# aosokin/os2d

Measured on AMD Instinct MI355X. Metric: query-image-pairs/s (1280-px input, ResNet50, N-class), higher is better.
Workload: dtype fftx3 (as fft; the per-bin complex GEMM on the fp16 MFMA with spectra split into fp16 hi+lo, 3 MFMAs per product, fp32 accumulate)

## Files before the change

os2d_amd/csrc/dft_mfma.h:

```cpp
#pragma once

#ifndef DFT_DEV
#error "the includer defines DFT_DEV, DFT_TID, DFT_BID, DFT_GRID, DFT_LDS, DFT_BARRIER, DFT_MFMA, DFT_SHFL_XOR, DFT_SHFL_XOR_U32, DFT_BALLOT, DFT_FLAG, DFT_FLAG_SET, DFT_RAISE, DFT_UNIFORM"
#endif

#ifndef DFT_HD
#define DFT_HD static inline
#endif
#ifndef DFT_MEMBER
#define DFT_MEMBER inline
#endif
#ifndef DFT_LANDED
#define DFT_LANDED(X)
#endif
#ifndef DFT_FWD_PREFETCH_AFTER
#define DFT_FWD_PREFETCH_AFTER 2
#endif
#ifndef DFT_INV_PREFETCH_AFTER
#define DFT_INV_PREFETCH_AFTER 2
#endif
#ifndef DFT_PIPE_REGA
#define DFT_PIPE_REGA 1
#endif
#ifndef DFT_PIPE_LDS
#define DFT_PIPE_LDS 1
#endif
#ifndef DFT_SCHED_FENCE
#define DFT_SCHED_FENCE()
#endif
#ifndef DFT_STREAM_STORE
#define DFT_STREAM_STORE(P, V) (*(P) = (V))
#endif
#ifndef DFT_STAMP
#define DFT_STAMP(K)
#define DFT_STAMP_BEGIN()
#define DFT_STAMP_END(BASE)
#endif

#include "tile_common.h"

namespace os2d_dft {

typedef float f32x4u __attribute__((ext_vector_type(4), aligned(4)));

constexpr int DFT_THR = 512, DFT_WAVES = 8;
constexpr int DFT_G = 4;
constexpr int DFT_MAXP = 64;
constexpr int DFT_MAXV = 48;
constexpr int DFT_MAXWK = 96;
constexpr int DFT_KREG = 8;
constexpr int DFT_OUT_SHB = 0, DFT_OUT_SHB_BORDERS = 1, DFT_OUT_PLANES = 2;

struct DftPlan {
  int H, W;
  int P, Q, V, NBINS;
  int T, TY, TX, TH, TW;
  int oy, ox;
  int LH, LW;
  int RH;
  int Pp;
  int Wk;
  int N1;
  int M2;
  int Mx;
  int N2;
  int MA;
  int MB;
  int KB;
  int NBo;
  int G;
  int eT;
  int fast;
  unsigned inv_cg, inv_t, inv_tx, inv_c4, inv_v, inv_pq, inv_og, inv_kg, inv_pp;
  int lds_const, lds_union, lds_total;
};

DFT_HD int dft_round_up(int x, int m) { return (x + m - 1) / m * m; }
DFT_HD unsigned dft_magic(unsigned d) { return d > 1 ? (unsigned)(((1ull << 32) + d - 1) / d) : 0u; }

DFT_HD int dft_units_fqt(int P, int Q) { return (dft_round_up(Q, 16) / 8) * 2 * dft_round_up(Q + 2, 32); }
constexpr int DFT_R2_P = 64, DFT_R2_MATU = 8 * 2 * 64, DFT_R2_TWU = 16;
constexpr int DFT_R2_LDS_TW = 512;
DFT_HD bool dft_radix2(int P) { return P == DFT_R2_P; }
DFT_HD int dft_units_fp2(int P, int Q) {
  return dft_radix2(P) ? DFT_R2_MATU + DFT_R2_TWU : (2 * dft_round_up(P, 8) / 8) * 2 * dft_round_up(2 * P, 32);
}
DFT_HD int dft_units_e2(int P, int Q) { return (2 * dft_round_up(P, 8) / 8) * 2 * dft_round_up(2 * P, 32); }
DFT_HD int dft_units_gq(int P, int Q) { return (dft_round_up(Q + 2, 16) / 8) * 2 * dft_round_up(Q, 32); }
DFT_HD size_t dft_matrices_units(int P, int Q) {
  return (size_t)dft_units_fqt(P, Q) + dft_units_fp2(P, Q) + dft_units_e2(P, Q) + dft_units_gq(P, Q);
}

static inline bool dft_plan_transform(int LH, int LW, int RH, int ncols, int minP, int minQ, int G, DftPlan* pl) {
  pl->G = G;
  pl->P = dft_round_up(minP, 4);
  if (pl->P == 60) pl->P = DFT_R2_P;
  pl->Q = dft_round_up(minQ, 2);
  pl->V = pl->Q / 2 + 1;
  pl->NBINS = dft_round_up(pl->P * pl->V, 8);
  pl->LH = LH;
  pl->LW = LW;
  pl->RH = RH;
  pl->Pp = dft_round_up(pl->P, 8);
  pl->Wk = dft_round_up(LW, 16);
  pl->N1 = dft_round_up(2 * pl->V, 32);
  pl->M2 = dft_round_up(2 * pl->P, 32);
  pl->Mx = dft_round_up(G * pl->Pp, 32);
  pl->N2 = dft_round_up(G * pl->V, 32);
  pl->MA = dft_round_up(2 * RH, 32);
  pl->MB = G * (pl->MA / 2);
  pl->KB = dft_round_up(2 * pl->V, 16);
  pl->NBo = dft_round_up(ncols, 32);
  int e = 0;
  while ((1 << e) < pl->P) ++e;
  pl->eT = e + 1;
  if (pl->P > DFT_MAXP || pl->V > DFT_MAXV || pl->Wk > DFT_MAXWK || LH > pl->P || LW > pl->Q || RH > pl->P) return false;
  const int fqt = (pl->Wk / 8) * 2 * pl->N1 * 16, gq = (pl->KB / 8) * 2 * pl->NBo * 16;
  const int x = (pl->Wk / 8) * 2 * (pl->Mx + 1) * 16, r2 = (2 * pl->Pp / 8) * 2 * (pl->N2 + 1) * 16;
  const int xs = pl->V * (pl->P * 8 * G + 16);
  const int y2 = r2, tt = (pl->KB / 8) * 2 * (pl->MB + 1) * 16;
  int u = x;
  if (r2 > u) u = r2;
  if (xs > u) u = xs;
  if (y2 > u) u = y2;
  if (tt > u) u = tt;
  if (G == 8) {
    if (dft_radix2(pl->P)) return false;
    const int fp2 = (2 * pl->Pp / 8) * 2 * pl->M2 * 16;
    const int ca = fqt + fp2, cb = gq + fp2;
    pl->lds_const = ca > cb ? ca : cb;
    pl->lds_union = dft_round_up(u, 256);
    pl->lds_total = pl->lds_const + pl->lds_union + 1024;
    const int t1 = (pl->Mx / 32) * (pl->N1 / 32), t2 = (pl->M2 / 32) * (pl->N2 / 32), tA = (pl->MA / 32) * (pl->N2 / 32),
              tB = (pl->MB / 32) * (pl->NBo / 32);
    const int npos = pl->Pp * (pl->Wk / 4), nitem = G * pl->V * (pl->Pp / 8);
    return pl->lds_total <= 160 * 1024 && t1 <= 24 && t2 <= 24 && tA <= 24 && tB <= 24 && npos <= 2 * DFT_THR && nitem <= 3 * DFT_THR;
  }
  pl->lds_const = fqt > gq ? fqt : gq;
  pl->lds_union = dft_round_up(u, 256);
  pl->lds_total = pl->lds_const + pl->lds_union + 1024;
  return pl->lds_total <= 160 * 1024;
}

static inline void dft_set_tiles(DftPlan* pl, int H, int W, int TY, int TX, int TH, int TW) {
  pl->H = H;
  pl->W = W;
  pl->TY = TY;
  pl->TX = TX;
  pl->T = TY * TX;
  pl->TH = TH;
  pl->TW = TW;
  pl->oy = TY > 1 ? 3 : 0;
  pl->ox = TX > 1 ? 3 : 0;
  pl->fast = (pl->T == 1 && (W & 3) == 0) ? 1 : 0;
  pl->inv_t = dft_magic((unsigned)pl->T);
  pl->inv_tx = dft_magic((unsigned)TX);
  pl->inv_c4 = dft_magic((unsigned)(pl->Wk / 4));
  pl->inv_v = dft_magic((unsigned)pl->V);
  pl->inv_pq = dft_magic((unsigned)(pl->P / 4 * pl->G * 2));
  pl->inv_kg = dft_magic((unsigned)(pl->Pp / 8));
  pl->inv_pp = dft_magic((unsigned)pl->Pp);
}

struct DftSize {
  int P, Q;
};
// ... 63 lines not shown
  *hi = __builtin_bit_cast(u32x2, h);
#ifdef DFT_SPLIT_LO_PAIR
  u32x2 l;
  l[0] = DFT_SPLIT_LO_PAIR(a, b, (*hi)[0]);
  l[1] = DFT_SPLIT_LO_PAIR(c, d, (*hi)[1]);
  *lo = l;
#else
  const half4 l = __builtin_convertvector(x - __builtin_convertvector(h, f32x4), half4);
  *lo = __builtin_bit_cast(u32x2, l);
#endif
}

DFT_DEV half8 dft_frag(const u32x4* p) { return __builtin_bit_cast(half8, *p); }

DFT_DEV f32x16 dft_mma3(half8 ah, half8 al, half8 bh, half8 bl, f32x16 acc) {
  acc = DFT_MFMA(ah, bl, acc);
  acc = DFT_MFMA(al, bh, acc);
  acc = DFT_MFMA(ah, bh, acc);
  return acc;
}

template <int NT, int KS>
DFT_DEV void dft_product_rega(f32x16* acc, const half8* ah, const half8* al, int ksn, const u32x4* B, int bstride, int nt0,
                              int ntstep, int l31, int hw) {
  constexpr int KR = KS ? KS : DFT_KREG;
  half8 bh[2][NT], bl[2][NT];
#define DFT_REGA_READ(KSTEP, SET)                                                                                          \
  _Pragma("unroll") for (int j = 0; j < NT; ++j) {                                                                         \
    bh[SET][j] = dft_frag(B + (size_t)((2 * (KSTEP) + hw) * 2 + 0) * bstride + (nt0 + ntstep * j) * 32 + l31);             \
    bl[SET][j] = dft_frag(B + (size_t)((2 * (KSTEP) + hw) * 2 + 1) * bstride + (nt0 + ntstep * j) * 32 + l31);             \
  }
  if (DFT_PIPE_REGA) DFT_REGA_READ(0, 0)
#pragma unroll
  for (int ks = 0; ks < KR; ++ks) {
    if (KS || ks < ksn) {
      if (DFT_PIPE_REGA) {
        if (ks + 1 < KR && (KS || ks + 1 < ksn)) DFT_REGA_READ(ks + 1, (ks + 1) & 1)
        DFT_SCHED_FENCE();
      } else {
        DFT_REGA_READ(ks, ks & 1)
      }
#pragma unroll
      for (int j = 0; j < NT; ++j) acc[j] = dft_mma3(ah[ks], al[ks], bh[ks & 1][j], bl[ks & 1][j], acc[j]);
      if (DFT_PIPE_REGA) DFT_SCHED_FENCE();
    }
  }
#undef DFT_REGA_READ
}

template <int KS>
DFT_DEV void dft_product_rega_any(f32x16* acc, int ntiles, const half8* ah, const half8* al, int ksn, const u32x4* B, int bstride,
                                  int nt0, int ntstep, int l31, int hw) {
  if (ntiles == 3) dft_product_rega<3, KS>(acc, ah, al, ksn, B, bstride, nt0, ntstep, l31, hw);
  else if (ntiles == 2) dft_product_rega<2, KS>(acc, ah, al, ksn, B, bstride, nt0, ntstep, l31, hw);
  else if (ntiles == 1) dft_product_rega<1, KS>(acc, ah, al, ksn, B, bstride, nt0, ntstep, l31, hw);
}

template <int NT, bool SHARE, int NW, int PIPE_MODE>
DFT_DEV void dft_product_lds(f32x16* acc, int ks0, int ks1, const u32x4* A, int astride, const u32x4* B, int bstride, int t0, int mtn,
                             int l31, int hw) {
  constexpr int NA = SHARE ? 1 : NT;
  int tm[NT], tn[NT];
#pragma unroll
  for (int j = 0; j < NT; ++j) {
    const int t = t0 + NW * j;
    tn[j] = t / mtn;
    tm[j] = t - tn[j] * mtn;
  }
  half8 ah[2][NA], al[2][NA], bh[2][NT], bl[2][NT];
#define DFT_LDS_READ(KSTEP, SET)                                                                                           \
  {                                                                                                                        \
    const int kc_ = (KSTEP) < ks1 ? (KSTEP) : ks1 - 1;                                                                     \
    _Pragma("unroll") for (int j = 0; j < NA; ++j) {                                                                       \
      ah[SET][j] = dft_frag(A + (size_t)((2 * kc_ + hw) * 2 + 0) * astride + tm[j] * 32 + l31);                            \
      al[SET][j] = dft_frag(A + (size_t)((2 * kc_ + hw) * 2 + 1) * astride + tm[j] * 32 + l31);                            \
    }                                                                                                                      \
    _Pragma("unroll") for (int j = 0; j < NT; ++j) {                                                                       \
      bh[SET][j] = dft_frag(B + (size_t)((2 * kc_ + hw) * 2 + 0) * bstride + tn[j] * 32 + l31);                            \
      bl[SET][j] = dft_frag(B + (size_t)((2 * kc_ + hw) * 2 + 1) * bstride + tn[j] * 32 + l31);                            \
    }                                                                                                                      \
  }
#define DFT_LDS_MMA(SET)                                                                                                   \
  DFT_SCHED_FENCE();                                                                                                       \
  _Pragma("unroll") for (int j = 0; j < NT; ++j)                                                                           \
    acc[j] = dft_mma3(ah[SET][SHARE ? 0 : j], al[SET][SHARE ? 0 : j], bh[SET][j], bl[SET][j], acc[j]);                    \
  DFT_SCHED_FENCE();
  if (ks0 >= ks1) return;
  constexpr bool PIPE = PIPE_MODE == 2 || (PIPE_MODE == 1 && SHARE);
  if (!PIPE) {
    for (int ks = ks0; ks < ks1; ++ks) {
      DFT_LDS_READ(ks, 0)
      _Pragma("unroll") for (int j = 0; j < NT; ++j)
        acc[j] = dft_mma3(ah[0][SHARE ? 0 : j], al[0][SHARE ? 0 : j], bh[0][j], bl[0][j], acc[j]);
    }
    return;
  }
  DFT_LDS_READ(ks0, 0)
  int ks = ks0;
  for (; ks + 1 < ks1; ks += 2) {
    DFT_LDS_READ(ks + 1, 1)
    DFT_LDS_MMA(0)
    DFT_LDS_READ(ks + 2, 0)
    DFT_LDS_MMA(1)
  }
  if (ks < ks1) {
    DFT_LDS_MMA(0)
  }
#undef DFT_LDS_READ
#undef DFT_LDS_MMA
}

template <int NW, int PIPE_MODE>
DFT_DEV void dft_product_lds_any(f32x16* acc, int ntiles, int ks0, int ks1, const u32x4* A, int astride, const u32x4* B, int bstride,
                                 int t0, int mtn, int l31, int hw) {
  const bool share = mtn == NW;
  if (ntiles == 3) {
    if (share) dft_product_lds<3, true, NW, PIPE_MODE>(acc, ks0, ks1, A, astride, B, bstride, t0, mtn, l31, hw);
    else dft_product_lds<3, false, NW, PIPE_MODE>(acc, ks0, ks1, A, astride, B, bstride, t0, mtn, l31, hw);
  } else if (ntiles == 2) {
    if (share) dft_product_lds<2, true, NW, PIPE_MODE>(acc, ks0, ks1, A, astride, B, bstride, t0, mtn, l31, hw);
    else dft_product_lds<2, false, NW, PIPE_MODE>(acc, ks0, ks1, A, astride, B, bstride, t0, mtn, l31, hw);
  } else if (ntiles == 1) {
    dft_product_lds<1, true, NW, PIPE_MODE>(acc, ks0, ks1, A, astride, B, bstride, t0, mtn, l31, hw);
  }
}

DFT_DEV void dft_matrix_unit(int which, int unit, int P, int Q, const double* twP, const double* twQ, u32x4* out) {
  const int V = Q / 2 + 1;
  const bool r2 = which == 1 && dft_radix2(P);
  if (r2 && unit >= DFT_R2_MATU) {
    const int u = 2 * (unit - DFT_R2_MATU);
    u32x4 o;
    for (int t = 0; t < 4; ++t) o[t] = __builtin_bit_cast(unsigned, (float)twP[2 * u + t]);
    *out = o;
    return;
  }
  const int tws = r2 ? 2 : 1;
  if (r2) P /= 2;
  const int Pp = dft_round_up(P, 8);
  int cols, kidx, hl, col;
  double vals[8];
  if (which == 0) cols = dft_round_up(2 * V, 32);
  else if (which == 1 || which == 2) cols = dft_round_up(2 * P, 32);
  else cols = dft_round_up(Q, 32);
  col = unit % cols;
  hl = (unit / cols) & 1;
  kidx = unit / (2 * cols);
  for (int t = 0; t < 8; ++t) {
    const int k = kidx * 8 + t;
    double x = 0.0;
    if (which == 0) {
      const int v = col >> 1, ri = col & 1;
      if (k < Q && v < V) x = twQ[2 * (int)(((long long)v * k) % Q) + ri] * 16384.0;
    } else if (which == 1) {
      const int ri = k / Pp, h = k - ri * Pp, u = col >> 1, ro = col & 1;
      if (h < P && u < P && ri < 2) {
        const int a = (int)(((long long)u * h) % P) * tws;
        const double c = twP[2 * a], s = -twP[2 * a + 1];
        x = (ro == 0 ? (ri == 0 ? c : s) : (ri == 0 ? -s : c)) * 16384.0;
      }
    } else if (which == 2) {
      const int ri = k / Pp, u = k - ri * Pp, h = col >> 1, ro = col & 1;
      if (u < P && h < P && ri < 2) {
        const int a = (int)(((long long)u * h) % P);
        const double c = twP[2 * a], s = -twP[2 * a + 1];
        x = (ro == 0 ? (ri == 0 ? c : -s) : (ri == 0 ? s : c)) * 16384.0;
      }
    } else {
      const int v = k >> 1, ri = k & 1;
      if (v < V && col < Q) {
        const double a = (v == 0 || 2 * v == Q) ? 1.0 : 2.0;
        x = a * twQ[2 * (int)(((long long)v * col) % Q) + ri] * 8192.0;
      }
    }
    vals[t] = x;
  }
  unsigned w[4];
  for (int t = 0; t < 4; ++t) {
    unsigned short b[2];
    for (int e = 0; e < 2; ++e) {
      const double x = vals[2 * t + e];
      const _Float16 h = (_Float16)x;
      const _Float16 r = hl == 0 ? h : (_Float16)(x - (double)h);
      b[e] = __builtin_bit_cast(unsigned short, r);
    }
    w[t] = (unsigned)b[0] | ((unsigned)b[1] << 16);
  }
  u32x4 o;
  o[0] = w[0];
  o[1] = w[1];
  o[2] = w[2];
  o[3] = w[3];
  *out = o;
}

template <bool TILED, bool FAST, int G, int NW, int KS2 = 0>
DFT_DEV void dft_forward_body(const float* corr,
                              const float* invn,
                              float* X,
                              const u32x4* FqT, const u32x4* Fp2, const DftPlan& pl, int C, int Cpad, int NBT, int iters) {
  constexpr int THR = NW * 64;
  constexpr bool ALDS = G == 8;
  constexpr bool R2 = !ALDS && KS2 == 8;
  unsigned char* smem = DFT_LDS;
  const int tid = DFT_TID, lane = tid & 63, l31 = lane & 31, hw = lane >> 5;
  const int wv = DFT_UNIFORM(tid >> 6);
  const int P = pl.P, V = pl.V, Pp = pl.Pp, Wk = pl.Wk, N1 = pl.N1, Mx = pl.Mx, N2 = pl.N2, LH = pl.LH, LW = pl.LW, W = pl.W, H = pl.H;
  const int MxS = Mx + 1, N2S = N2 + 1;
  const int CG = (C + G - 1) / G, HW = H * W;
  const bool unit_norm = invn == nullptr;
  u32x4* ldsF = reinterpret_cast<u32x4*>(smem);
  u32x4* ldsU = reinterpret_cast<u32x4*>(smem + pl.lds_const);
  unsigned char* ldsUb = smem + pl.lds_const;
  const int nF = (Wk / 8) * 2 * N1;
  for (int i = tid; i < nF; i += THR) ldsF[i] = FqT[i];
  const unsigned char* ldsTw = smem + pl.lds_const + pl.lds_union + DFT_R2_LDS_TW;
  if (R2 && tid < DFT_R2_TWU) reinterpret_cast<u32x4*>(smem + pl.lds_const + pl.lds_union + DFT_R2_LDS_TW)[tid] = Fp2[DFT_R2_MATU + tid];
  u32x4* ldsP = ldsF + nF;
  if (ALDS)
    for (int i = tid; i < (2 * Pp / 8) * 2 * pl.M2; i += THR) ldsP[i] = Fp2[i];

  const int mt1n = Mx / 32, nt1n = N1 / 32, nt2n = N2 / 32, mt2n = pl.M2 / 32;
  const int ks1n = Wk / 16, ks2n = 2 * Pp / 16;
  const int mt2 = wv & 3;
  constexpr int KR2 = R2 ? 4 : KS2 ? KS2 : DFT_KREG;
  half8 fp2h[KR2], fp2l[KR2];
  if (R2) {
#pragma unroll
    for (int ks = 0; ks < KR2; ++ks) {
      fp2h[ks] = dft_frag(Fp2 + ((size_t)((2 * ks + hw) * 2 + 0)) * 64 + (mt2 & 1) * 32 + l31);
      fp2l[ks] = dft_frag(Fp2 + ((size_t)((2 * ks + hw) * 2 + 1)) * 64 + (mt2 & 1) * 32 + l31);
    }
  } else if (!ALDS) {
#pragma unroll
    for (int ks = 0; ks < KR2; ++ks) {
      const int kc = ks < ks2n ? ks : 0, mc = mt2 < mt2n ? mt2 : 0;
      fp2h[ks] = dft_frag(Fp2 + ((size_t)((2 * kc + hw) * 2 + 0)) * pl.M2 + mc * 32 + l31);
      fp2l[ks] = dft_frag(Fp2 + ((size_t)((2 * kc + hw) * 2 + 1)) * pl.M2 + mc * 32 + l31);
    }
  }
  if (!ALDS) {
#pragma unroll
    for (int ks = 0; ks < KR2; ++ks) {
      DFT_LANDED(fp2h[ks]);
      DFT_LANDED(fp2l[ks]);
    }
  }

  constexpr int NSLOT = ALDS ? 2 : 3 * 512 / THR;
  const int npos = Pp * (Wk / 4);
  f32x4 pc[NSLOT][G], pn[NSLOT];
#define DFT_FWD_ITER(IT)                                                                                     \
  const int pr_ = dft_div((IT), pl.inv_cg), cg_ = (IT)-pr_ * CG;                                             \
  const int nb_ = TILED ? dft_div(pr_, pl.inv_t) : pr_, tile_ = TILED ? pr_ - nb_ * pl.T : 0;               \
  const int ty_ = TILED ? dft_div(tile_, pl.inv_tx) : 0, tx_ = TILED ? tile_ - ty_ * pl.TX : 0;             \
  const int Y0 = TILED ? ty_ * pl.TH - pl.oy : 0, X0 = TILED ? tx_ * pl.TW - pl.ox : 0;                     \
  const int c0_ = cg_ * G;
#define DFT_FWD_POS(TID, S)                                                                                  \
  const int i_ = (TID) + (S)*THR;                                                                        \
  const int r_ = dft_div(i_, pl.inv_c4), c4_ = i_ - r_ * (Wk / 4);                                          \
  const int y_ = Y0 + r_, x_ = X0 + 4 * c4_;
#define DFT_FWD_PREFETCH(IT, TID) DFT_FWD_PREFETCH_SLOTS(IT, TID, 0, NSLOT)
#define DFT_FWD_PREFETCH_SLOTS(IT, TID, S0, S1)                                                              \
  {                                                                                                          \
    DFT_FWD_ITER(IT)                                                                                         \
     \
    const float* nrm_ = invn ? invn + (size_t)nb_ * HW : corr + ((size_t)nb_ * C + (c0_ < C ? c0_ : C - 1)) * HW; \
    _Pragma("unroll") for (int s = (S0); s < (S1); ++s) {                                                    \
      DFT_FWD_POS(TID, s)                                                                                    \
      if (FAST) {                                                                                            \
        const bool ok = i_ < npos && r_ < LH && 4 * c4_ < LW;                                                \
        const int off = ok ? y_ * W + x_ : 0;                                                                \
        pn[s] = *reinterpret_cast<const f32x4*>(nrm_ + off);                                                \
        _Pragma("unroll") for (int g = 0; g < G; ++g) {                                                  \
          const int c = c0_ + g < C ? c0_ + g : C - 1;                                                       \
          pc[s][g] = *reinterpret_cast<const f32x4*>(corr + ((size_t)nb_ * C + c) * HW + off);              \
        }                                                                                                    \
      } else {                                                                                               \
                                                                           \
        const bool rok = i_ < npos && r_ < LH && y_ >= 0 && y_ < H;                                          \
        const int off0 = y_ * W + x_;                                                                        \
        const bool vec = rok && off0 >= 0 && off0 + 3 < HW;                                                  \
        const int offv = vec ? off0 : 0;                                                                     \
        pn[s] = *reinterpret_cast<const f32x4u*>(nrm_ + offv);                                               \
        _Pragma("unroll") for (int g = 0; g < G; ++g) {                                                      \
          const int c = c0_ + g < C ? c0_ + g : C - 1;                                                       \
          pc[s][g] = *reinterpret_cast<const f32x4u*>(corr + ((size_t)nb_ * C + c) * HW + offv);             \
        }                                                                                                    \
        if (rok && !vec) {                                                                                   \
          _Pragma("unroll") for (int e = 0; e < 4; ++e) {                                                    \
            const bool ok = 4 * c4_ + e < LW && x_ + e >= 0 && x_ + e < W;                                   \
            const int off = ok ? y_ * W + x_ + e : 0;                                                        \
            pn[s][e] = nrm_[off];                                                                            \
            _Pragma("unroll") for (int g = 0; g < G; ++g) {                                                  \
              const int c = c0_ + g < C ? c0_ + g : C - 1;                                                   \
              pc[s][g][e] = corr[((size_t)nb_ * C + c) * HW + off];                                          \
            }                                                                                                \
          }                                                                                                  \
        }                                                                                                    \
      }                                                                                                      \
    }                                                                                                        \
  }
  const int first = (DFT_GRID & 7) == 0 ? (DFT_BID & 7) * (DFT_GRID >> 3) + (DFT_BID >> 3) : DFT_BID;
  if (first < iters) DFT_FWD_PREFETCH(first, tid)
  DFT_BARRIER();

  DFT_STAMP_BEGIN()
  for (int it = first; it < iters; it += DFT_GRID) {
    int tl = tid;
#ifndef OS2D_HOST_EMU
    asm volatile("" : "+v"(tl));
#endif
    const int lane = tl & 63, l31 = lane & 31, hw = lane >> 5;
    DFT_FWD_ITER(it)
    {
#pragma unroll
      for (int s = 0; s < NSLOT; ++s) {
        DFT_FWD_POS(tl, s)
        if (i_ < npos) {
          float nsc[4];
#pragma unroll
          for (int e = 0; e < 4; ++e) {
            const bool ok = FAST ? (r_ < LH && 4 * c4_ < LW) : (r_ < LH && y_ >= 0 && y_ < H && 4 * c4_ + e < LW && x_ + e >= 0 && x_ + e < W);
            nsc[e] = ok ? (unit_norm ? 32768.0f : pn[s][e] * 32768.0f) : 0.f;
          }
#pragma unroll
          for (int g = 0; g < G; ++g) {
            u32x2 hi = {0u, 0u}, lo = {0u, 0u};
            if (c0_ + g < C)
              dft_split4(fmaxf(pc[s][g][0], 0.f) * nsc[0], fmaxf(pc[s][g][1], 0.f) * nsc[1], fmaxf(pc[s][g][2], 0.f) * nsc[2],
                         fmaxf(pc[s][g][3], 0.f) * nsc[3], &hi, &lo);
            const int m = g * Pp + (R2 ? (r_ & 1) * 32 + (r_ >> 1) : r_);
            unsigned char* dst = ldsUb + ((size_t)((c4_ >> 1) * 2) * MxS + m) * 16 + (c4_ & 1) * 8;
            *reinterpret_cast<u32x2*>(dst) = hi;
            *reinterpret_cast<u32x2*>(dst + (size_t)MxS * 16) = lo;
          }
        }
      }
      for (int i = tid; i < (Mx - G * Pp) * (Wk / 8) * 2; i += THR) {
        const int m = G * Pp + i % (Mx - G * Pp), kh = i / (Mx - G * Pp);
        ldsU[(size_t)kh * MxS + m] = u32x4{0u, 0u, 0u, 0u};
      }
    }
    DFT_BARRIER();
    DFT_STAMP(0)

    f32x16 acc[3];
    int tm[3], tn[3];
    int nt1w = 0;
#pragma unroll
    for (int j = 0; j < 3; ++j) {
      const int t = wv + NW * j;
      const bool mine = t < mt1n * nt1n;
      tn[j] = mine ? t / mt1n : 0;
      tm[j] = mine ? t - tn[j] * mt1n : -1;
      nt1w += mine ? 1 : 0;
#pragma unroll
      for (int r = 0; r < 16; ++r) acc[j][r] = 0.f;
    }
    dft_product_lds_any<NW, DFT_PIPE_LDS ? 2 : 0>(acc, nt1w, 0, ks1n, ldsU, MxS, ldsF, N1, wv, mt1n, l31, hw);
    DFT_BARRIER();
    DFT_STAMP(1)

#pragma unroll
    for (int j = 0; j < 3; ++j) {
      if (tm[j] < 0) continue;
      const int n = tn[j] * 32 + l31, v = n >> 1, ri = n & 1;
#pragma unroll
      for (int q = 0; q < 4; ++q) {
        const int mb = tm[j] * 32 + 8 * q;
        const int img = dft_div(mb, pl.inv_pp), h0 = mb - img * Pp + 4 * hw;
        if (v < V && img < G) {
          u32x2 hi, lo;
          const float sc = 1.0f / 2097152.0f;
          dft_split4(acc[j][4 * q] * sc, acc[j][4 * q + 1] * sc, acc[j][4 * q + 2] * sc, acc[j][4 * q + 3] * sc, &hi, &lo);
          const int kg = R2 ? (h0 >> 5) * 8 + ri * 4 + ((h0 & 31) >> 3) : ri * (Pp / 8) + (h0 >> 3);
          unsigned char* dst = ldsUb + ((size_t)(kg * 2) * N2S + img * V + v) * 16 + (h0 & 4) * 2;
          *reinterpret_cast<u32x2*>(dst) = hi;
          *reinterpret_cast<u32x2*>(dst + (size_t)N2S * 16) = lo;
        }
      }
    }
    DFT_BARRIER();
    DFT_STAMP(2)

    f32x16 xc[3];
    int un[3], um[3];
    int nt2w = 0;
#pragma unroll
    for (int j = 0; j < 3; ++j) {
      const int t = wv + NW * j;
      const int nt = ALDS ? t / mt2n : (wv >> 2) + (NW / 4) * j;
      const bool mine = ALDS ? t < mt2n * nt2n : (nt < nt2n && mt2 < mt2n);
      un[j] = mine ? nt : -1;
      um[j] = ALDS ? t - nt * mt2n : mt2;
      nt2w += mine ? 1 : 0;
#pragma unroll
      for (int r = 0; r < 16; ++r) xc[j][r] = 0.f;
    }
    const int itn = it + DFT_GRID < iters ? it + DFT_GRID : it;
    {
      if (ALDS) {
        dft_product_lds_any<NW, DFT_PIPE_LDS ? 2 : 0>(xc, nt2w, 0, ks2n, ldsP, pl.M2, ldsU, N2S, wv, mt2n, l31, hw);
        DFT_FWD_PREFETCH_SLOTS(itn, tl, 0, NSLOT)
      } else if (!R2 && (DFT_FWD_PREFETCH_AFTER == 1 || (DFT_FWD_PREFETCH_AFTER == 2 && KS2 > 0 && KS2 <= 6))) {
        dft_product_rega_any<KS2>(xc, nt2w, fp2h, fp2l, ks2n, ldsU, N2S, wv >> 2, NW / 4, l31, hw);
        DFT_FWD_PREFETCH_SLOTS(itn, tl, 0, NSLOT)
      } else if (R2) {
        DFT_FWD_PREFETCH_SLOTS(itn, tl, 0, NSLOT)
        dft_product_rega_any<4>(xc, nt2w, fp2h, fp2l, 4, ldsU + (size_t)(mt2 >> 1) * 16 * N2S, N2S, wv >> 2, NW / 4, l31, hw);
      } else {
        DFT_FWD_PREFETCH_SLOTS(itn, tl, 0, NSLOT)
        dft_product_rega_any<KS2>(xc, nt2w, fp2h, fp2l, ks2n, ldsU, N2S, wv >> 2, NW / 4, l31, hw);
      }
    }
    DFT_BARRIER();
    DFT_STAMP(3)

    const int XS = P * 8 * G + 16;
#pragma unroll
    for (int j = 0; j < 3; ++j) {
      if (un[j] < 0) continue;
      const int n2 = un[j] * 32 + l31;
      const int img = dft_div(n2, pl.inv_v), v = n2 - img * V;
#pragma unroll
      for (int q = 0; q < 4; ++q) {
        const int u0 = (um[j] * 32 + 8 * q + 4 * hw) >> 1;
        if (img < G && u0 < P) {
          const float sc = 1.0f / 4194304.0f;
          f32x4 o;
          o[0] = xc[j][4 * q] * sc;
          o[1] = xc[j][4 * q + 1] * sc;
          o[2] = xc[j][4 * q + 2] * sc;
          o[3] = xc[j][4 * q + 3] * sc;
          *reinterpret_cast<f32x4*>(ldsUb + (size_t)v * XS + (u0 >> 2) * (G * 32) + img * 32 + (u0 & 3) * 8) = o;
        }
      }
    }
    DFT_BARRIER();
    DFT_STAMP(4)

    {
      const int per_v = (P / 4) * (G * 2), npieces = V * per_v;
      size_t qstride;
      float* dstbase = X + dft_spectra_pair0(pr_, NBT, pl.NBINS / 4, Cpad, &qstride) + (size_t)c0_ * 8;
      if (R2) {
        constexpr int per_h = (DFT_R2_P / 8) * (G * 2);
        for (int i = tl; i < V * per_h; i += THR) {
          const int v = i / per_h, rem = i - v * per_h;
          const int uq = rem / (2 * G), jj = rem - uq * (2 * G);
          const unsigned char* src = ldsUb + (size_t)v * XS + uq * (G * 32) + jj * 16;
          const f32x4 e = *reinterpret_cast<const f32x4*>(src);
          const f32x4 o = *reinterpret_cast<const f32x4*>(src + (DFT_R2_P / 8) * (G * 32));
          const f32x4 w = *reinterpret_cast<const f32x4*>(ldsTw + (4 * uq + 2 * (jj & 1)) * 8);
          f32x4 t;
          t[0] = w[0] * o[0] - w[1] * o[1];
          t[1] = w[0] * o[1] + w[1] * o[0];
          t[2] = w[2] * o[2] - w[3] * o[3];
          t[3] = w[2] * o[3] + w[3] * o[2];
          float* dst = dstbase + (size_t)(v * (P / 4) + uq) * qstride + jj * 4;
          DFT_STREAM_STORE(reinterpret_cast<f32x4*>(dst), e + t);
          DFT_STREAM_STORE(reinterpret_cast<f32x4*>(dst + (size_t)(DFT_R2_P / 8) * qstride), e - t);
        }
      } else
      for (int i = tl; i < npieces; i += THR) {
        const int v = dft_div(i, pl.inv_pq), rem = i - v * per_v;
        const int uq = rem / (2 * G), jj = rem - uq * (2 * G);
        const f32x4 val = *reinterpret_cast<const f32x4*>(ldsUb + (size_t)v * XS + uq * (G * 32) + jj * 16);
        DFT_STREAM_STORE(reinterpret_cast<f32x4*>(dstbase + (size_t)(v * (P / 4) + uq) * qstride + jj * 4), val);
      }
      const int qpad0 = (P * V) / 4, qpad1 = pl.NBINS / 4;
      for (int i = tl; i < (qpad1 - qpad0) * 2 * G; i += THR)
        *reinterpret_cast<f32x4*>(dstbase + (size_t)(qpad0 + i / (2 * G)) * qstride + (i % (2 * G)) * 4) = f32x4{0.f, 0.f, 0.f, 0.f};
    }
    DFT_BARRIER();
    DFT_STAMP(5)
  }
  DFT_STAMP_END(0)
#undef DFT_FWD_ITER
#undef DFT_FWD_POS
#undef DFT_FWD_PREFETCH
#undef DFT_FWD_PREFETCH_SLOTS
}

template <bool TILED, int KSA = 0, int G = DFT_G>
DFT_DEV void dft_inverse_body(const float* Y,
                              const float* bp,
                              int MTP, unsigned char* out,
                              const u32x4* E2, const u32x4* Gq, const DftPlan& pl, int Cout, int NBT, int PLANE, int Ws,
                              int BASE, int iters, DFT_FLAG bad_flag, int zero_borders) {
  unsigned char* smem = DFT_LDS;
  const int tid = DFT_TID, lane = tid & 63, l31 = lane & 31, hw = lane >> 5;
  const int wv = DFT_UNIFORM(tid >> 6);
  const int P = pl.P, V = pl.V, Pp = pl.Pp, N2 = pl.N2, MB = pl.MB, KB = pl.KB, NBo = pl.NBo, H = pl.H, W = pl.W;
  const int N2S = N2 + 1, MBS = MB + 1;
  const int OG = Cout / G;
  constexpr bool ALDS = G == 8;
  constexpr int LG = G == 8 ? 3 : 2;
  u32x4* ldsG = reinterpret_cast<u32x4*>(smem);
  u32x4* ldsU = reinterpret_cast<u32x4*>(smem + pl.lds_const);
  unsigned char* ldsUb = smem + pl.lds_const;
  float* smaxw = reinterpret_cast<float*>(smem + pl.lds_const + pl.lds_union);
  const int nG = (KB / 8) * 2 * NBo, NQ = dft_round_up(pl.Q, 32);
  for (int i = tid; i < nG; i += DFT_THR) {
    const int kh = i / NBo, n = i - kh * NBo;
    ldsG[i] = Gq[(size_t)kh * NQ + n];
  }
  const int MAfull = dft_round_up(2 * P, 32);
  u32x4* ldsE = ldsG + nG;
  if (ALDS)
    for (int i = tid; i < (2 * Pp / 8) * 2 * MAfull; i += DFT_THR) ldsE[i] = E2[i];

  const int mtAn = pl.MA / 32, ntAn = N2 / 32, ksAn = 2 * Pp / 16;
  const int mtBn = MB / 32, ntBn = NBo / 32, ksBn = KB / 16;
  const int mtA = wv & 3;
  constexpr int KRA = KSA ? KSA : DFT_KREG;
  half8 e2h[KRA], e2l[KRA];
  if (!ALDS) {
#pragma unroll
    for (int ks = 0; ks < KRA; ++ks) {
      const int kc = ks < ksAn ? ks : 0, mc = mtA < mtAn ? mtA : 0;
      e2h[ks] = dft_frag(E2 + ((size_t)((2 * kc + hw) * 2 + 0)) * MAfull + mc * 32 + l31);
      e2l[ks] = dft_frag(E2 + ((size_t)((2 * kc + hw) * 2 + 1)) * MAfull + mc * 32 + l31);
    }
#pragma unroll
    for (int ks = 0; ks < KRA; ++ks) {
      DFT_LANDED(e2h[ks]);
      DFT_LANDED(e2l[ks]);
    }
  }

  constexpr int NITEM = 3;
  const int uoct = Pp / 8, nitem = G * V * uoct;
  f32x4 py[NITEM][4];
#define DFT_INV_PREFETCH(IT, TID) DFT_INV_PREFETCH_ITEMS(IT, TID, 0, NITEM)
#define DFT_INV_PREFETCH_ITEMS(IT, TID, S0, S1)                                             \
  {                                                                                         \
    const int pr_ = dft_div((IT), pl.inv_og), og_ = (IT)-pr_ * OG;                          \
    size_t qstride;                                                                         \
    const float* src_ = Y + dft_spectra_pair0(pr_, NBT, pl.NBINS / 4, Cout, &qstride) + (size_t)og_ * G * 8; \
    _Pragma("unroll") for (int s = (S0); s < (S1); ++s) {                                   \
      const int e_ = (TID) + s * DFT_THR;                                                   \
      const int ec_ = e_ < nitem ? e_ : 0;                                                  \
      const int pimg_ = ec_ & (G - 1), prest_ = ec_ >> LG;                                  \
      const int pv_ = dft_div(prest_, pl.inv_kg), puo_ = prest_ - pv_ * (Pp / 8);           \
      const int q0_ = pv_ * (P / 4) + 2 * puo_;                                             \
      const bool ptwo_ = 8 * puo_ + 4 < P;                                                  \
      const float* p0_ = src_ + (size_t)q0_ * qstride + pimg_ * 8;                          \
      const float* p1_ = src_ + (size_t)(ptwo_ ? q0_ + 1 : q0_) * qstride + pimg_ * 8;      \
      py[s][0] = *reinterpret_cast<const f32x4*>(p0_);                                     \
      py[s][1] = *reinterpret_cast<const f32x4*>(p0_ + 4);                                 \
      py[s][2] = *reinterpret_cast<const f32x4*>(p1_);                                     \
      py[s][3] = *reinterpret_cast<const f32x4*>(p1_ + 4);                                 \
    }                                                                                       \
  }
#define DFT_INV_ITEM(E)                                                                     \
  const int img_ = (E) & (G - 1), rest_ = (E) >> LG;                                        \
  const int v_ = dft_div(rest_, pl.inv_kg), uo_ = rest_ - v_ * uoct;                        \
  const bool two_ = 8 * uo_ + 4 < P;
#define DFT_INV_MAXIMA(TID)                                                                 \
  {                                                                                         \
    float m = 0.f;                                                                          \
    _Pragma("unroll") for (int s = 0; s < NITEM; ++s)                                       \
      if ((TID) + s * DFT_THR < nitem) {                                                    \
        DFT_INV_ITEM((TID) + s * DFT_THR)                                                   \
        (void)img_;                                                                         \
        (void)v_;                                                                           \
        (void)uo_;                                                                          \
        _Pragma("unroll") for (int k = 0; k < 4; ++k)                                       \
          if (k < 2 || two_) {                                                              \
            _Pragma("unroll") for (int e = 0; e < 4; ++e) m = fmaxf(m, fabsf(py[s][k][e])); \
          }                                                                                 \
      }                                                                                     \
    if (G == 4) m = fmaxf(m, DFT_SHFL_XOR(m, 4));                                           \
    m = fmaxf(m, DFT_SHFL_XOR(m, 8));                                                       \
    m = fmaxf(m, DFT_SHFL_XOR(m, 16));                                                      \
    m = fmaxf(m, DFT_SHFL_XOR(m, 32));                                                      \
    if (lane < G) smaxw[wv * G + lane] = m;                                                 \
  }
  bool bad = false;
  const int first = (DFT_GRID & 7) == 0 ? (DFT_BID & 7) * (DFT_GRID >> 3) + (DFT_BID >> 3) : DFT_BID;
  if (first < iters) {
    DFT_INV_PREFETCH(first, tid)
    DFT_INV_MAXIMA(tid)
  }
  DFT_BARRIER();

  DFT_STAMP_BEGIN()
  for (int it = first; it < iters; it += DFT_GRID) {
    int tl = tid;
#ifndef OS2D_HOST_EMU
    asm volatile("" : "+v"(tl));
#endif
    const int lane = tl & 63, l31 = lane & 31, hw = lane >> 5;
    const int pr = dft_div(it, pl.inv_og), og = it - pr * OG;
// ... 224 lines not shown
```

os2d_amd/csrc/dft_mfma.hip:

```cpp
#include "tile_common.h"
#include <map>
#include <mutex>
#include <utility>

extern __shared__ __attribute__((aligned(16))) unsigned char os2d_dft_smem[];

#define DFT_DEV __device__ __forceinline__
#define DFT_HD __host__ __device__ static inline
#define DFT_MEMBER __device__ __forceinline__
#define DFT_TID ((int)threadIdx.x)
#define DFT_BID ((int)blockIdx.x)
#define DFT_GRID ((int)gridDim.x)
#define DFT_LDS os2d_dft_smem
#define DFT_BARRIER() asm volatile("s_waitcnt lgkmcnt(0)\n\ts_barrier" ::: "memory")
#define DFT_MFMA(a, b, c) __builtin_amdgcn_mfma_f32_32x32x16_f16(a, b, c, 0, 0, 0)
#define DFT_SHFL_XOR(v, m) __shfl_xor(v, m, 64)
#define DFT_SHFL_XOR_U32(v, m) ((unsigned)__shfl_xor((int)(v), m, 64))
#define DFT_BALLOT(p) __builtin_amdgcn_ballot_w64(p)
#define DFT_UNIFORM(x) __builtin_amdgcn_readfirstlane(x)
#define DFT_SCHED_FENCE() __builtin_amdgcn_sched_barrier(0)
#define DFT_LANDED(X) asm volatile("" : "+v"(X))
#define DFT_SPLIT_LO_PAIR(a, b, hi) os2d_split_lo_pair(a, b, hi)
#define DFT_STREAM_STORE(P, V) os2d_stream_store(P, V)
#define DFT_FLAG Os2dRangeFlag
#define DFT_FLAG_SET(f) ((f).word != nullptr)
#define DFT_RAISE(f) os2d_raise(f)
#ifdef OS2D_DIAG_DFT_STAMPS
__device__ unsigned long long os2d_dft_stamps[16];
#define DFT_STAMP_BEGIN() unsigned long long st_acc_[6] = {0, 0, 0, 0, 0, 0}, st_n_ = 0, st_last_ = wall_clock64();
#define DFT_STAMP(K)                                   \
  {                                                    \
    const unsigned long long t_ = wall_clock64();      \
    st_acc_[K] += t_ - st_last_;                       \
    st_last_ = t_;                                     \
    if ((K) == 5) ++st_n_;                             \
  }
#define DFT_STAMP_END(BASE)                                                                   \
  if (threadIdx.x == 0) {                                                                     \
    for (int k_ = 0; k_ < 6; ++k_) atomicAdd(&os2d_dft_stamps[(BASE) + k_], st_acc_[k_]);     \
    atomicAdd(&os2d_dft_stamps[(BASE) + 6], st_n_);                                           \
  }
#endif
#include "dft_mfma.h"

namespace {

using namespace os2d_dft;

template <bool TILED, bool FAST, int G, int NW, int KS>
__global__ __launch_bounds__(NW * 64, 8 / NW) void dft_forward_kernel(const float* __restrict__ corr, const float* __restrict__ invn,
                                                                      float* __restrict__ X, const u32x4* __restrict__ FqT,
                                                                      const u32x4* __restrict__ Fp2, DftPlan pl, int C, int Cpad, int NBT,
                                                                      int iters) {
  dft_forward_body<TILED, FAST, G, NW, KS>(corr, invn, X, FqT, Fp2, pl, C, Cpad, NBT, iters);
}

template <bool TILED, int KS, int G>
__global__ __launch_bounds__(DFT_THR, 1) void dft_inverse_kernel(const float* __restrict__ Y, const float* __restrict__ bp, int MTP,
                                                                 unsigned char* __restrict__ out, const u32x4* __restrict__ E2,
                                                                 const u32x4* __restrict__ Gq, DftPlan pl, int Cout, int NBT, int PLANE,
                                                                 int Ws, int BASE, int iters, Os2dRangeFlag status, int zero_borders) {
  dft_inverse_body<TILED, KS, G>(Y, bp, MTP, out, E2, Gq, pl, Cout, NBT, PLANE, Ws, BASE, iters, status, zero_borders);
}

typedef void (*dft_forward_fn)(const float*, const float*, float*, const u32x4*, const u32x4*, DftPlan, int, int, int, int);
typedef void (*dft_inverse_fn)(const float*, const float*, int, unsigned char*, const u32x4*, const u32x4*, DftPlan, int, int, int, int, int,
                               int, Os2dRangeFlag, int);
template <int G, int NW, int KS>
dft_forward_fn dft_forward_variant(const DftPlan& pl) {
  return pl.T > 1 ? dft_forward_kernel<true, false, G, NW, KS> : (pl.fast ? dft_forward_kernel<false, true, G, NW, KS> : dft_forward_kernel<false, false, G, NW, KS>);
}
template <int G, int NW>
dft_forward_fn dft_forward_pick(const DftPlan& pl) {
  if constexpr (G == 8) {
    return dft_forward_variant<G, NW, 0>(pl);
  } else {
    switch (2 * pl.Pp / 16) {
      case 5: return dft_forward_variant<G, NW, 5>(pl);
      case 6: return dft_forward_variant<G, NW, 6>(pl);
      case 7: return dft_forward_variant<G, NW, 7>(pl);
      case 8: return dft_forward_variant<G, NW, 8>(pl);
      default: return dft_forward_variant<G, NW, 0>(pl);
    }
  }
}
template <int KS, int G = DFT_G>
dft_inverse_fn dft_inverse_variant(const DftPlan& pl) {
  return pl.T > 1 ? dft_inverse_kernel<true, KS, G> : dft_inverse_kernel<false, KS, G>;
}
dft_inverse_fn dft_inverse_pick(const DftPlan& pl) {
  if (pl.G == 8) return dft_inverse_variant<0, 8>(pl);
  switch (2 * pl.Pp / 16) {
    case 5: return dft_inverse_variant<5>(pl);
    case 6: return dft_inverse_variant<6>(pl);
    case 7: return dft_inverse_variant<7>(pl);
    case 8: return dft_inverse_variant<8>(pl);
    default: return dft_inverse_variant<0>(pl);
  }
}

__global__ __launch_bounds__(256) void dft_matrices_kernel(const double* __restrict__ twP, const double* __restrict__ twQ, int P, int Q,
                                                           u32x4* __restrict__ out) {
  const int n0 = dft_units_fqt(P, Q), n1 = n0 + dft_units_fp2(P, Q), n2 = n1 + dft_units_e2(P, Q), n3 = n2 + dft_units_gq(P, Q);
  const int i = blockIdx.x * 256 + threadIdx.x;
  if (i >= n3) return;
  const int which = i < n0 ? 0 : i < n1 ? 1 : i < n2 ? 2 : 3;
  const int base = which == 0 ? 0 : which == 1 ? n0 : which == 2 ? n1 : n2;
  dft_matrix_unit(which, i - base, P, Q, twP, twQ, out + i);
}

bool dft_plan_cached(int H, int W, DftPlan* out, bool g8 = true) {
  static const bool g8_enabled = [] {
    const char* e = getenv("OS2D_DFT_G8");
    return !(e && e[0] == '0');
  }();
  struct Entry {
    bool ok, ok8;
    DftPlan pl, pl8;
  };
  static std::mutex mu;
  static std::map<std::pair<int, int>, Entry> cache;
  {
    std::lock_guard<std::mutex> lock(mu);
    auto it = cache.find({H, W});
    if (it != cache.end()) {
      if (it->second.ok) *out = (g8 && g8_enabled && it->second.ok8) ? it->second.pl8 : it->second.pl;
      return it->second.ok;
    }
  }
  Entry e = {};
  e.ok = dft_make_plan(H, W, &e.pl);
  e.ok8 = e.ok && dft_plan_g8(e.pl, &e.pl8);
  if (e.ok) *out = (g8 && g8_enabled && e.ok8) ? e.pl8 : e.pl;
  std::lock_guard<std::mutex> lock(mu);
  if (cache.size() >= 4096) cache.clear();
  cache[{H, W}] = e;
  return e.ok;
}

int dft_grid(int iters, int per_cu = 1) {
  int g = iters < 256 * per_cu ? iters : 256 * per_cu;
  return os2d_round_up(g, 8);
}

}

int os2d_dft_plan(int H, int W, int* P, int* Q, int* nbins, int* tiles) {
  DftPlan pl;
  if (H < 1 || W < 1 || !dft_plan_cached(H, W, &pl)) return 0;
  if (P) *P = pl.P;
  if (Q) *Q = pl.Q;
  if (nbins) *nbins = pl.NBINS;
  if (tiles) {
    tiles[0] = pl.TY;
    tiles[1] = pl.TX;
    tiles[2] = pl.TH;
    tiles[3] = pl.TW;
    tiles[4] = pl.LH;
    tiles[5] = pl.LW;
  }
  return 1;
}

size_t os2d_dft_matrices_size(int P, int Q) { return dft_matrices_units(P, Q) * 16; }

int os2d_launch_dft_matrices(const double* twP64, const double* twQ64, int P, int Q, void* out, hipStream_t stream) {
  if (P < 4 || (P & 3) || P > DFT_MAXP || Q < 2 || (Q & 1) || Q / 2 + 1 > DFT_MAXV) {
    os2d_set_error("dft_matrices: transform %d x %d is outside the kernels' range (P %% 4 == 0, P <= %d, Q even, Q/2 + 1 <= %d)", P, Q,
                   DFT_MAXP, DFT_MAXV);
    return -3;
// ... 71 lines not shown
```

Measured before the change: 48640.

## Fuse radix-2 row DFT stages in registers, skipping LDS round trip

For the R2 path, the first-stage accumulators are split into fp16 hi/lo fragments held in registers and fed directly as MFMA B operands to a cosine and a sine product. The real/imaginary recombination uses a DPP lane swap instead of a shuffle. This removes the intermediate LDS write, a barrier, and the LDS reads of the second product. The twiddle matrix layout changes to separate cos/sin fragments, which costs extra registers and an extra MFMA set per tile, and the prefetch is moved earlier.

```diff
diff --git a/os2d_amd/csrc/dft_mfma.h b/os2d_amd/csrc/dft_mfma.h
--- a/os2d_amd/csrc/dft_mfma.h
+++ b/os2d_amd/csrc/dft_mfma.h
@@ -12,6 +12,9 @@
 #endif
 #ifndef DFT_LANDED
 #define DFT_LANDED(X)
+#endif
+#ifndef DFT_SWAP1
+#define DFT_SWAP1(V) DFT_SHFL_XOR(V, 1)
 #endif
 #ifndef DFT_FWD_PREFETCH_AFTER
 #define DFT_FWD_PREFETCH_AFTER 2
@@ -381,6 +384,12 @@
     if (which == 0) {
       const int v = col >> 1, ri = col & 1;
       if (k < Q && v < V) x = twQ[2 * (int)(((long long)v * k) % Q) + ri] * 16384.0;
+    } else if (r2) {
+      const int h = 8 * (2 * (kidx >> 1) + (t >> 2)) + 4 * (kidx & 1) + (t & 3), u = col & 31;
+      if (kidx < 4) {
+        const int a = (int)(((long long)u * h) % P) * tws;
+        x = (col < 32 ? twP[2 * a] : -twP[2 * a + 1]) * 16384.0;
+      }
     } else if (which == 1) {
       const int ri = k / Pp, h = k - ri * Pp, u = col >> 1, ro = col & 1;
       if (h < P && u < P && ri < 2) {
@@ -456,9 +465,9 @@
   half8 fp2h[KR2], fp2l[KR2];
   if (R2) {
 #pragma unroll
-    for (int ks = 0; ks < KR2; ++ks) {
-      fp2h[ks] = dft_frag(Fp2 + ((size_t)((2 * ks + hw) * 2 + 0)) * 64 + (mt2 & 1) * 32 + l31);
-      fp2l[ks] = dft_frag(Fp2 + ((size_t)((2 * ks + hw) * 2 + 1)) * 64 + (mt2 & 1) * 32 + l31);
+    for (int f = 0; f < KR2; ++f) {
+      fp2h[f] = dft_frag(Fp2 + ((size_t)((2 * (f & 1) + hw) * 2 + 0)) * 64 + (f >> 1) * 32 + l31);
+      fp2l[f] = dft_frag(Fp2 + ((size_t)((2 * (f & 1) + hw) * 2 + 1)) * 64 + (f >> 1) * 32 + l31);
     }
   } else if (!ALDS) {
 #pragma unroll
@@ -591,85 +600,129 @@
     DFT_BARRIER();
     DFT_STAMP(1)
 
-#pragma unroll
-    for (int j = 0; j < 3; ++j) {
-      if (tm[j] < 0) continue;
-      const int n = tn[j] * 32 + l31, v = n >> 1, ri = n & 1;
-#pragma unroll
-      for (int q = 0; q < 4; ++q) {
-        const int mb = tm[j] * 32 + 8 * q;
-        const int img = dft_div(mb, pl.inv_pp), h0 = mb - img * Pp + 4 * hw;
-        if (v < V && img < G) {
-          u32x2 hi, lo;
+    if constexpr (R2) {
+      const int img = wv >> 1, par = wv & 1;
+      half8 bh[3][2], bl[3][2];
+#pragma unroll
+      for (int j = 0; j < 3; ++j) {
+#pragma unroll
+        for (int a = 0; a < 2; ++a) {
           const float sc = 1.0f / 2097152.0f;
-          dft_split4(acc[j][4 * q] * sc, acc[j][4 * q + 1] * sc, acc[j][4 * q + 2] * sc, acc[j][4 * q + 3] * sc, &hi, &lo);
-          const int kg = R2 ? (h0 >> 5) * 8 + ri * 4 + ((h0 & 31) >> 3) : ri * (Pp / 8) + (h0 >> 3);
-          unsigned char* dst = ldsUb + ((size_t)(kg * 2) * N2S + img * V + v) * 16 + (h0 & 4) * 2;
-          *reinterpret_cast<u32x2*>(dst) = hi;
-          *reinterpret_cast<u32x2*>(dst + (size_t)N2S * 16) = lo;
-        }
-      }
-    }
-    DFT_BARRIER();
-    DFT_STAMP(2)
-
-    f32x16 xc[3];
-    int un[3], um[3];
-    int nt2w = 0;
-#pragma unroll
-    for (int j = 0; j < 3; ++j) {
-      const int t = wv + NW * j;
-      const int nt = ALDS ? t / mt2n : (wv >> 2) + (NW / 4) * j;
-      const bool mine = ALDS ? t < mt2n * nt2n : (nt < nt2n && mt2 < mt2n);
-      un[j] = mine ? nt : -1;
-      um[j] = ALDS ? t - nt * mt2n : mt2;
-      nt2w += mine ? 1 : 0;
-#pragma unroll
-      for (int r = 0; r < 16; ++r) xc[j][r] = 0.f;
-    }
-    const int itn = it + DFT_GRID < iters ? it + DFT_GRID : it;
+          u32x2 h0, l0, h1, l1;
+          dft_split4(acc[j][8 * a] * sc, acc[j][8 * a + 1] * sc, acc[j][8 * a + 2] * sc, acc[j][8 * a + 3] * sc, &h0, &l0);
+          dft_split4(acc[j][8 * a + 4] * sc, acc[j][8 * a + 5] * sc, acc[j][8 * a + 6] * sc, acc[j][8 * a + 7] * sc, &h1, &l1);
+          bh[j][a] = __builtin_bit_cast(half8, u32x4{h0[0], h0[1], h1[0], h1[1]});
+          bl[j][a] = __builtin_bit_cast(half8, u32x4{l0[0], l0[1], l1[0], l1[1]});
+        }
+      }
+      const int itn = it + DFT_GRID < iters ? it + DFT_GRID : it;
+      DFT_FWD_PREFETCH_SLOTS(itn, tl, 0, NSLOT)
+      const int XS = P * 8 * G + 16;
+      const float sc2 = 1.0f / 4194304.0f, sg = (l31 & 1) ? -sc2 : sc2;
+#pragma unroll
+      for (int j = 0; j < 3; ++j) {
+        f32x16 cr, sr;
+#pragma unroll
+        for (int r = 0; r < 16; ++r) cr[r] = sr[r] = 0.f;
+#pragma unroll
+        for (int a = 0; a < 2; ++a) {
+          cr = dft_mma3(fp2h[a], fp2l[a], bh[j][a], bl[j][a], cr);
+          sr = dft_mma3(fp2h[2 + a], fp2l[2 + a], bh[j][a], bl[j][a], sr);
+        }
+        float z[16];
+#pragma unroll
+        for (int r = 0; r < 16; ++r) {
+          z[r] = cr[r] * sc2 + DFT_SWAP1(sr[r]) * sg;
+          DFT_LANDED(z[r]);
+        }
+        const int n = j * 32 + l31, v = n >> 1;
+        if (v < V) {
+          unsigned char* dst = ldsUb + (size_t)v * XS + (par * (DFT_R2_P / 8) + hw) * (G * 32) + img * 32 + (n & 1) * 4;
+#pragma unroll
+          for (int r = 0; r < 16; ++r) *reinterpret_cast<float*>(dst + (r >> 2) * (2 * G * 32) + (r & 3) * 8) = z[r];
+        }
+      }
+      DFT_BARRIER();
+      DFT_STAMP(3)
+    } else {
+#pragma unroll
+      for (int j = 0; j < 3; ++j) {
+        if (tm[j] < 0) continue;
+        const int n = tn[j] * 32 + l31, v = n >> 1, ri = n & 1;
+#pragma unroll
+        for (int q = 0; q < 4; ++q) {
+          const int mb = tm[j] * 32 + 8 * q;
+          const int img = dft_div(mb, pl.inv_pp), h0 = mb - img * Pp + 4 * hw;
+          if (v < V && img < G) {
+            u32x2 hi, lo;
+            const float sc = 1.0f / 2097152.0f;
+            dft_split4(acc[j][4 * q] * sc, acc[j][4 * q + 1] * sc, acc[j][4 * q + 2] * sc, acc[j][4 * q + 3] * sc, &hi, &lo);
+            const int kg = ri * (Pp / 8) + (h0 >> 3);
+            unsigned char* dst = ldsUb + ((size_t)(kg * 2) * N2S + img * V + v) * 16 + (h0 & 4) * 2;
+            *reinterpret_cast<u32x2*>(dst) = hi;
+            *reinterpret_cast<u32x2*>(dst + (size_t)N2S * 16) = lo;
+          }
+        }
+      }
+      DFT_BARRIER();
+      DFT_STAMP(2)
+
+      f32x16 xc[3];
+      int un[3], um[3];
+      int nt2w = 0;
+#pragma unroll
+      for (int j = 0; j < 3; ++j) {
+        const int t = wv + NW * j;
+        const int nt = ALDS ? t / mt2n : (wv >> 2) + (NW / 4) * j;
+        const bool mine = ALDS ? t < mt2n * nt2n : (nt < nt2n && mt2 < mt2n);
+        un[j] = mine ? nt : -1;
+        um[j] = ALDS ? t - nt * mt2n : mt2;
+        nt2w += mine ? 1 : 0;
+#pragma unroll
+        for (int r = 0; r < 16; ++r) xc[j][r] = 0.f;
+      }
+      const int itn = it + DFT_GRID < iters ? it + DFT_GRID : it;
+      {
+        if (ALDS) {
+          dft_product_lds_any<NW, DFT_PIPE_LDS ? 2 : 0>(xc, nt2w, 0, ks2n, ldsP, pl.M2, ldsU, N2S, wv, mt2n, l31, hw);
+          DFT_FWD_PREFETCH_SLOTS(itn, tl, 0, NSLOT)
+        } else if (DFT_FWD_PREFETCH_AFTER == 1 || (DFT_FWD_PREFETCH_AFTER == 2 && KS2 > 0 && KS2 <= 6)) {
+          dft_product_rega_any<KS2>(xc, nt2w, fp2h, fp2l, ks2n, ldsU, N2S, wv >> 2, NW / 4, l31, hw);
+          DFT_FWD_PREFETCH_SLOTS(itn, tl, 0, NSLOT)
+        } else {
+          DFT_FWD_PREFETCH_SLOTS(itn, tl, 0, NSLOT)
+          dft_product_rega_any<KS2>(xc, nt2w, fp2h, fp2l, ks2n, ldsU, N2S, wv >> 2, NW / 4, l31, hw);
+        }
+      }
+      DFT_BARRIER();
+      DFT_STAMP(3)
+
+      const int XS = P * 8 * G + 16;
+#pragma unroll
+      for (int j = 0; j < 3; ++j) {
+        if (un[j] < 0) continue;
+        const int n2 = un[j] * 32 + l31;
+        const int img = dft_div(n2, pl.inv_v), v = n2 - img * V;
+#pragma unroll
+        for (int q = 0; q < 4; ++q) {
+          const int u0 = (um[j] * 32 + 8 * q + 4 * hw) >> 1;
+          if (img < G && u0 < P) {
+            const float sc = 1.0f / 4194304.0f;
+            f32x4 o;
+            o[0] = xc[j][4 * q] * sc;
+            o[1] = xc[j][4 * q + 1] * sc;
+            o[2] = xc[j][4 * q + 2] * sc;
+            o[3] = xc[j][4 * q + 3] * sc;
+            *reinterpret_cast<f32x4*>(ldsUb + (size_t)v * XS + (u0 >> 2) * (G * 32) + img * 32 + (u0 & 3) * 8) = o;
+          }
+        }
+      }
+      DFT_BARRIER();
+      DFT_STAMP(4)
+    }
+
     {
-      if (ALDS) {
-        dft_product_lds_any<NW, DFT_PIPE_LDS ? 2 : 0>(xc, nt2w, 0, ks2n, ldsP, pl.M2, ldsU, N2S, wv, mt2n, l31, hw);
-        DFT_FWD_PREFETCH_SLOTS(itn, tl, 0, NSLOT)
-      } else if (!R2 && (DFT_FWD_PREFETCH_AFTER == 1 || (DFT_FWD_PREFETCH_AFTER == 2 && KS2 > 0 && KS2 <= 6))) {
-        dft_product_rega_any<KS2>(xc, nt2w, fp2h, fp2l, ks2n, ldsU, N2S, wv >> 2, NW / 4, l31, hw);
-        DFT_FWD_PREFETCH_SLOTS(itn, tl, 0, NSLOT)
-      } else if (R2) {
-        DFT_FWD_PREFETCH_SLOTS(itn, tl, 0, NSLOT)
-        dft_product_rega_any<4>(xc, nt2w, fp2h, fp2l, 4, ldsU + (size_t)(mt2 >> 1) * 16 * N2S, N2S, wv >> 2, NW / 4, l31, hw);
-      } else {
-        DFT_FWD_PREFETCH_SLOTS(itn, tl, 0, NSLOT)
-        dft_product_rega_any<KS2>(xc, nt2w, fp2h, fp2l, ks2n, ldsU, N2S, wv >> 2, NW / 4, l31, hw);
-      }
-    }
-    DFT_BARRIER();
-    DFT_STAMP(3)
-
-    const int XS = P * 8 * G + 16;
-#pragma unroll
-    for (int j = 0; j < 3; ++j) {
-      if (un[j] < 0) continue;
-      const int n2 = un[j] * 32 + l31;
-      const int img = dft_div(n2, pl.inv_v), v = n2 - img * V;
-#pragma unroll
-      for (int q = 0; q < 4; ++q) {
-        const int u0 = (um[j] * 32 + 8 * q + 4 * hw) >> 1;
-        if (img < G && u0 < P) {
-          const float sc = 1.0f / 4194304.0f;
-          f32x4 o;
-          o[0] = xc[j][4 * q] * sc;
-          o[1] = xc[j][4 * q + 1] * sc;
-          o[2] = xc[j][4 * q + 2] * sc;
-          o[3] = xc[j][4 * q + 3] * sc;
-          *reinterpret_cast<f32x4*>(ldsUb + (size_t)v * XS + (u0 >> 2) * (G * 32) + img * 32 + (u0 & 3) * 8) = o;
-        }
-      }
-    }
-    DFT_BARRIER();
-    DFT_STAMP(4)
-
-    {
+      const int XS = P * 8 * G + 16;
       const int per_v = (P / 4) * (G * 2), npieces = V * per_v;
       size_t qstride;
       float* dstbase = X + dft_spectra_pair0(pr_, NBT, pl.NBINS / 4, Cpad, &qstride) + (size_t)c0_ * 8;
diff --git a/os2d_amd/csrc/dft_mfma.hip b/os2d_amd/csrc/dft_mfma.hip
--- a/os2d_amd/csrc/dft_mfma.hip
+++ b/os2d_amd/csrc/dft_mfma.hip
@@ -16,6 +16,7 @@
 #define DFT_MFMA(a, b, c) __builtin_amdgcn_mfma_f32_32x32x16_f16(a, b, c, 0, 0, 0)
 #define DFT_SHFL_XOR(v, m) __shfl_xor(v, m, 64)
 #define DFT_SHFL_XOR_U32(v, m) ((unsigned)__shfl_xor((int)(v), m, 64))
+#define DFT_SWAP1(v) __builtin_bit_cast(float, __builtin_amdgcn_update_dpp(0, __builtin_bit_cast(int, (float)(v)), 0xB1, 0xF, 0xF, true))
 #define DFT_BALLOT(p) __builtin_amdgcn_ballot_w64(p)
 #define DFT_UNIFORM(x) __builtin_amdgcn_readfirstlane(x)
 #define DFT_SCHED_FENCE() __builtin_amdgcn_sched_barrier(0)
```

After: 50190, median of 6. 1.03x the previous value.
